# eugenelet/CRFP

Hardware: AMD Instinct MI355X
Metric: sr_frames_per_sec (higher is better)
Workload: dtype f32; 1 GPU; BASELINE configs[1]: single MI355X, 7-frame 180x320 -> 1440x2560 x8 SR, batch=1, fp32, sigma_T=10; mode=clip, frames_per_clip=7, fv_size=96, clips_per_call=1, calls_in_flight_per_gpu=1, clips_in_flight_per_gpu=1, batching=one clip per call, storage=f32, parallelism=clip-sharded x1

## Files before the change

crfp_amd/csrc/engine.hip:

```cpp
#include "crfp_common.h"

#include <cstdlib>
#include <algorithm>
#include <cstring>
#include <mutex>
#include <string>
#include <unordered_map>
#include <vector>

namespace CRFP_NS {

struct ConvDef { const char* stem; int cout, cin; };
constexpr int kNumDsvConvs = 59, kNumCraConvs = 72;
static const ConvDef kConvs[kNumCraConvs] = {
    {"spynet.encoder1.0", 32, 6}, {"spynet.encoder1.2", 32, 32}, {"spynet.encoder2.0", 64, 32},
    {"spynet.encoder2.2", 64, 64}, {"spynet.encoder3.0", 128, 64}, {"spynet.encoder3.2", 128, 128},
    {"spynet.decoder1.0", 256, 128}, {"spynet.decoder1.2", 256, 256}, {"spynet.decoder2.0", 128, 256},
    {"spynet.decoder2.2", 128, 128}, {"spynet.decoder3.0", 64, 128}, {"spynet.decoder3.2", 64, 64},
    {"spynet.flow.0", 32, 64}, {"spynet.flow.2", 2, 32},
    {"dcn_0.dcn_block.0", 32, 66}, {"dcn_0.dcn_block.2", 32, 32}, {"dcn_0.dcn_offset", 144, 32},
    {"dcn_0.dcn_mask", 72, 32}, {"dcn_0.dcn", 32, 32},
    {"dcn_1.conv_fuse", 32, 64}, {"dcn_1.dcn_block.0", 32, 66}, {"dcn_1.dcn_block.2", 32, 32},
    {"dcn_1.dcn_offset", 144, 32}, {"dcn_1.dcn_mask", 72, 32}, {"dcn_1.dcn", 32, 32},
    {"dcn_2.conv_fuse", 32, 64}, {"dcn_2.dcn_block.0", 32, 66}, {"dcn_2.dcn_block.2", 32, 32},
// ... 296 lines not shown
struct Q4 {
    float* p = nullptr;
    int nq = 0, H = 0, W = 0;
    long long bs() const { return (long long)nq * H * W * 4; }
};

constexpr int kFlatFrames = 32, kChunkFrames = 8;

struct Layout {
    Arena A;
    int B, t, h, w;
    bool flat;
    int TC;
    Ten status, state_hr, carry;
    Ten flow_lr, e_lr0, x_lr, lr_q4, lr_keep[2];
    Ten fa0, fa1, fp1, fb0, fb1, fp2, fc0, fc1, fp3, fd0, fd1, fu1, fe0, fe1, fu2, ff0, ff1, fu3, fg0, fg1;
    Ten xin8[2], eh[2], x_hr[2], prop0[2], prop_a, prop_b, flow2[2], flow8[2], prev2, prev2w, prevhrw, carryw, fa, fb, offfeat[3], offmask,
        aligned, y0, y1, up, poff, g0, g1, g2, om3, al3, z0, z1, feat, fg2, sc_prop, sc_cw, sc_al, sc_up, sc_al3;
    Ten c_s1, c_a, c_b, c_lv[2][3], c_y, c_f;
    bool cra;
    int pq;
    Ten gate[2];
    long long gate_b;
    int h1, w1, h2, w2, h3, w3;
    int fnet_cap;
    Ten fpart;

    Layout(int B_, int t_, int h_, int w_, int wiring = W_DSV) : B(B_), t(t_), h(h_), w(w_), cra(wiring == W_CRA), pq(wiring >= W_SIMPLE ? 8 : 6) {
        flat = (long long)B * t <= kFlatFrames;
        TC = flat ? t : kChunkFrames;
        const int nb = t == 1 ? B : (flat ? B * t - 1 : TC);
        fnet_cap = nb;
        const int H2 = 2 * h, W2 = 2 * w, H8 = 8 * h, W8 = 8 * w;
        h1 = h / 2; w1 = w / 2; h2 = h1 / 2; w2 = w1 / 2; h3 = h2 / 2; w3 = w2 / 2;
        status = A.take("status", 1, 0, 1, B > 64 ? (B + 1) / 2 : 32, 1);
        state_hr = A.take("state_hr", B, 1, H8, W8, 0, 1);
        carry = A.take("carry", B, 6, H2, W2, 0, 1);
        flow_lr = A.take("flow_lr", t == 1 ? 2 * B : B * TC, 1, h, w, 0, 0, true);
// ... 25 lines not shown
        {
            const int lh[7] = {h, h1, h2, h3, 2 * h3, 4 * h3, 8 * h3}, lw[7] = {w, w1, w2, w3, 2 * w3, 4 * w3, 8 * w3};
            long long most = 0;
            for (int i = 0; i < 14; ++i) {
                const int kq = (kConvs[i].cin / 4 + 3) / 4 * 4, H = lh[i / 2], W = lw[i / 2];
                const int ks = H > 0 && W > 0 ? conv_auto_ksplit(H, W, (kConvs[i].cout + 31) / 32, kq) : 1;
                if (ks > 1) most = std::max(most, (long long)ks * kConvs[i].cout * H * W);
            }
            const long long per = (long long)h * w * 4;
            fpart = A.take("fnet.part", nb, (int)((most + per - 1) / per), h, w, 0, 0, true);
        }
        for (int p = 0; p < 2; ++p) {
            xin8[p] = A.take(p ? "xin8.1" : "xin8", B, 2, H8, W8);
            eh[p] = A.take(p ? "enc_hr0.1" : "enc_hr0", B, 1, H8, W8);
            x_hr[p] = A.take(p ? "x_hr.1" : "x_hr", B, 1, H8, W8);
            prop0[p] = A.take(p ? "prop0.1" : "prop0", B, pq, H2, W2);
            flow2[p] = A.take(p ? "flow2.1" : "flow2", B, 0, H2, W2, 1);
            flow8[p] = A.take(p ? "flow8.1" : "flow8", B, 0, H8, W8, 1);
            const int gtiles = ((W8 + 63) / 64) * ((H8 + 15) / 16);
            gate_b = ((long long)gtiles * 4 + 7) / 8 * 8;
            gate[p] = A.take(p ? "gate.1" : "gate", B, 0, 1, (int)(gate_b / 8), 1);
        }
        prop_a = A.take("prop_a", B, pq, H2, W2);
        prop_b = A.take("prop_b", B, pq, H2, W2);
        prev2 = A.take("prev2", B, 8, H2, W2, 0, 1);
        prev2w = A.take("prev2w", B, 8, H2, W2);
        prevhrw = A.take("prevhrw", B, 1, H8, W8);
        carryw = A.take("carryw", B, 6, H2, W2);
        fa = A.take("dcn.fa", B, 8, H2, W2);
        fb = A.take("dcn.fb", B, 8, H2, W2);
        for (int l = 0; l < 3; ++l) offfeat[l] = A.take(l == 0 ? "offfeat0" : (l == 1 ? "offfeat1" : "offfeat2"), B, 8, H2, W2);
        offmask = A.take("offmask", B, 54, H2, W2, 0, 0, true);
        aligned = A.take("aligned", B, 8, H2, W2);
        y0 = A.take("res.y0", B, 8, H2, W2);
        y1 = A.take("res.y1", B, 8, H2, W2);
        up = A.take("up", B, 1, H8, W8);
// ... 15 lines not shown
                for (int k = 0; k < 3; ++k) c_lv[p][k] = A.take(lvn[p][k], B, 4, H2, W2);
            c_y = A.take("cra.y", B, 8, H2, W2);
            c_f = A.take("cra.fused", B, 8, H2, W2);
        }
        if (t == 1 && B == 1) {
            fg2 = A.take("fg2", 1, 0, H2 / 2, W2, 1);
            sc_prop = A.take("fg.prop", 1, 6, H2, W2);
            sc_cw = A.take("fg.carry", 1, 2, H2, W2);
            sc_al = A.take("fg.aligned", 1, 8, H2, W2);
            sc_up = A.take("fg.up", 1, 1, H8, W8);
            sc_al3 = A.take("fg.aligned3", 1, 1, H8, W8);
        }
    }
    size_t bytes() const { return A.cur; }
    long long slot(int b, int i) const { return (long long)b * TC + i % TC; }
};

struct StreamCtx {
    unsigned n = 0;
    bool kept = false;
    bool chained = false;
};
struct SideStream {
    hipStream_t s = nullptr;
    std::vector<hipEvent_t> ev;
    std::unordered_map<const void*, StreamCtx> ctx;
    bool ok = true;
    hipEvent_t event(size_t i) {
        while (ev.size() <= i) {
            hipEvent_t e;
// ... 52 lines not shown
    int dev = 0;
    if (hipGetDevice(&dev) != hipSuccess || dev < 0 || dev >= kMaxDevices) return nullptr;
    return &side_table()[dev];
}
static SideStream* side_stream() {
    SideStream* ss = side_slot();
    if (!ss) return nullptr;
    if (!ss->s && ss->ok && hipStreamCreateWithFlags(&ss->s, hipStreamNonBlocking) != hipSuccess) ss->ok = false;
    return ss->ok ? ss : nullptr;
}
static bool side_stream_enabled() {
    static const bool on = !(getenv("CRFP_SIDE_STREAM") && atoi(getenv("CRFP_SIDE_STREAM")) == 0);
    return on;
}

struct Runner {
    const Model& M;
    const float* packed;
    char* ws;
    const Layout& L;
    hipStream_t s;
    int rc = 0;
    int strict = 0;
    bool down_done = false;
    int flow_slot = 0;
    float* flow_lr_slot() const { return F(L.flow_lr) + (long long)flow_slot * L.B * L.h * L.w * 4; }

    int ovf_div = 1, ovf_add = 0, ovf_off = 0, ovf_skip0 = 0;
    unsigned* ovf() const {
        static const bool env_strict = precision_env_strict(0);
// ... 74 lines not shown
        if (rc) return;
        const ConvArgs a = bind(idA, N, H, W, srcsA, {}), b = bind(idB, N, H, W, {{nullptr, 0}}, dstsB, residB, residB_bs);
        rc = launch_conv_pair(a, b, name, s);
    }
#endif
    bool pair_convs() const {
        static const int mode = !kActBf16 ? 0 : (getenv("CRFP_CONV_PAIR") ? atoi(getenv("CRFP_CONV_PAIR")) : 1);
        const long long pair_tiles = (long long)L.B * ((2 * L.w + 61) / 62) * ((2 * L.h + 7) / 8);
        return mode == 2 || (mode == 1 && pair_tiles <= 512);
    }
    void mfma_q(int id, int N, const Q4& in, const Q4& out) {
        mfma(id, N, in.H, in.W, {{in.p, in.bs()}}, {{out.p, out.bs(), 0, out.nq}});
    }
    struct NB { const float* p = nullptr; long long bs = 0; NB() {} NB(const float* p_, long long bs_) : p(p_), bs(bs_) {} };
    void narrow(int id, int H, int W, std::vector<NB> srcs, NB dst, NB resid = NB(), NB flow = NB(), const uint8_t* mask = nullptr,
                long long mask_bs = 0, int src0_pad = 0, int dst_pad = 0, NB base_lr = NB(), int gate_par = -1, int gate_h = 0, NB dst2 = NB()) {
        if (rc) return;
        const Item& it = M.items[id];
        NarrowArgs a = it.nw;
        for (size_t i = 0; i < srcs.size(); ++i) { a.src[i].p = srcs[i].p; a.src[i].bstride = srcs[i].bs; a.src[i].pad = 0; }
        a.src[0].pad = src0_pad;
        a.dst_pad = dst_pad;
        a.N = L.B; a.H = H; a.W = W;
        a.dst = const_cast<float*>(dst.p); a.dst_bstride = dst.bs;
        a.resid = resid.p; a.resid_bstride = resid.bs;
        a.flow = flow.p; a.flow_bstride = flow.bs;
        a.base = nullptr; a.base_lr = base_lr.p; a.base_bstride = base_lr.bs;
        a.mask = mask; a.mask_bstride = mask_bs;
        a.wpk = packed + it.off_w;
        a.bpk = packed + it.off_b;
        a.ovf = ovf(); a.ovf_div = ovf_div; a.ovf_add = ovf_add;
        a.dst2 = const_cast<float*>(dst2.p); a.dst2_bstride = dst2.bs;
        if (gate_par >= 0 && mask_gate_enabled()) { a.gate = gate_ptr(gate_par); a.gate_bstride = L.gate_b; a.gate_h = gate_h; }
        rc = launch_narrow(a, it.name, s);
    }
    void narrow_pair(int idA, int idB, const char* name, int H, int W, std::vector<NB> srcsA, NB dst, NB residB = NB(), NB flowB = NB(), NB dst2B = NB()) {
        if (rc) return;
        NarrowArgs a = M.items[idA].nw, b = M.items[idB].nw;
        for (size_t i = 0; i < srcsA.size(); ++i) { a.src[i].p = srcsA[i].p; a.src[i].bstride = srcsA[i].bs; a.src[i].pad = 0; }
        a.N = b.N = L.B; a.H = b.H = H; a.W = b.W = W;
        a.wpk = packed + M.items[idA].off_w; a.bpk = packed + M.items[idA].off_b;
        b.wpk = packed + M.items[idB].off_w; b.bpk = packed + M.items[idB].off_b;
        b.dst = const_cast<float*>(dst.p); b.dst_bstride = dst.bs;
        b.resid = residB.p; b.resid_bstride = residB.bs;
        b.flow = flowB.p; b.flow_bstride = flowB.bs;
        b.dst_pad = 0;
        b.dst2 = const_cast<float*>(dst2B.p); b.dst2_bstride = dst2B.bs;
        b.ovf = ovf(); b.ovf_div = ovf_div; b.ovf_add = ovf_add;
// ... 33 lines not shown
#endif
#ifdef CRFP_LAB
    static bool state_from_epilogue() {
        static const bool on = getenv("CRFP_STATE_FROM_EPILOGUE") ? atoi(getenv("CRFP_STATE_FROM_EPILOGUE")) != 0 : CRFP_STATE_FROM_EPILOGUE != 0;
        return on;
    }
#else
    static constexpr bool state_from_epilogue() { return CRFP_STATE_FROM_EPILOGUE != 0; }
#endif
#define RUN(expr) do { if (!rc) rc = (expr); } while (0)

    static bool mask_gate_enabled() {
        static const bool on = !(getenv("CRFP_MASK_GATE") && atoi(getenv("CRFP_MASK_GATE")) == 0);
        return on;
    }
    const uint8_t* gate_ptr(int par) const { return reinterpret_cast<const uint8_t*>(ws + L.gate[par]); }

    const float* lr_to_q4(const float* lrs, int n, int s0, int check_div = -1) {
        if (kActBf16) return lrs;
        float* dst = adv(F(L.lr_q4), (long long)s0 * L.h * L.w * 4);
        RUN(launch_nchw_to_q4(lrs, dst, n, 3, L.h, L.w, 0, s, check_div >= 0 ? ovf() : nullptr, check_div));
        return dst;
    }
    long long lr_frame_floats() const { return kActBf16 ? 3LL * L.h * L.w : (long long)L.h * L.w * 4 * (long long)sizeof(act_t) / 4; }
    long long lr_bs(long long nchw_bs) const { return kActBf16 ? nchw_bs : (nchw_bs ? (long long)L.h * L.w * 4 : 0); }

    void fnet(int nb, const float* cur, long long cur_bs, const float* prev, long long prev_bs, float* flow_out, int group = 0) {
        const int h = L.h, w = L.w;
        if (!rc && nb > L.fnet_cap) { set_error("dsv: FNet pass of %d pairs exceeds the workspace's %d", nb, L.fnet_cap); rc = CRFP_E_WORKSPACE; }
        if (rc || nb < 1) return;
        cur_bs = lr_bs(cur_bs); prev_bs = lr_bs(prev_bs);
// ... 38 lines not shown
        pool(conv(5, c0, c1), c1, p3);
        reduce(conv(6, p3, d0), d0);
        resize2(conv(7, d0, d1), d1, u1);
        reduce(conv(8, u1, e0), e0);
        resize2(conv(9, e0, e1), e1, u2);
        reduce(conv(10, u2, f0), f0);
        resize2(conv(11, f0, f1), f1, u3);
        reduce(conv(12, u3, g0), g0);
        mfma(IT_F0 + 13, nb, g0.H, g0.W, {{g0.p, g0.bs()}}, {{g1.p, g1.bs(), 0, g1.nq}}, 0, 0, nullptr, 0, nullptr, 0, nullptr, 0, 1);
        RUN(crfp::launch_upsample_q4(g1.p, g1.bs(), fl.p, fl.bs(), nb, 1, g1.H, g1.W, h, w, (float)g1.H / (float)h,
                                     (float)g1.W / (float)w, 1.0f, s, group));
    }

    void reset_state() {
        if (!rc && hipMemsetAsync(ws + L.status, 0, L.A.find(L.status.off)->bytes, s) != hipSuccess) { set_error("dsv: hipMemsetAsync of the status words failed"); rc = 1; }
        for (size_t off : {L.state_hr.off, L.carry.off, L.prev2.off}) {
            const Buf* b = L.A.find(off);
            if (!rc && hipMemsetAsync(ws + off - b->guard, 0, b->bytes + b->guard, s) != hipSuccess) {
                set_error("dsv: hipMemsetAsync of recurrent state failed");
                rc = 1;
            }
        }
    }

    void encode_lr(int n, const float* lrs, long long bs, long long slot0 = 0) {
        if (rc || n < 1) return;
        const long long xq = 8LL * L.h * L.w * 4;
        Q4 e0 = q(L.e_lr0, 8, L.h, L.w), x = q(L.x_lr, 8, L.h, L.w);
        e0.p = adv(e0.p, slot0 * xq); x.p = adv(x.p, slot0 * xq);
        mfma(IT_ENC_LR0, n, L.h, L.w, {{lrs, lr_bs(bs)}}, {{e0.p, e0.bs(), 0, 8}});
        mfma_q(IT_ENC_LR1, n, e0, x);
    }

    void clip_stage(const float* lq, int i0, int i1, int parts) {
        const long long lqf = lr_frame_floats(), lr_f = 3LL * L.h * L.w, fq = (long long)L.h * L.w * 4;
        const int t = L.t, B = L.B;
        struct Restore { Runner& r; int d, a, o; ~Restore() { r.ovf_div = d; r.ovf_add = a; r.ovf_off = o; r.ovf_skip0 = 0; } } restore{*this, ovf_div, ovf_add, ovf_off};
// ... 46 lines not shown
        const float* x_lr = nullptr; long long x_b = 0;
    };
    FrameIO frame_io(int i, const float* lrs, const float* fvs, const uint8_t* mks, float* out, int y_only) const {
        const long long lr_f = 3LL * L.h * L.w, hr_px = 64LL * L.h * L.w, xq = 8LL * L.h * L.w * 4, fq = (long long)L.h * L.w * 4;
        const int co = y_only ? 1 : 3, t = L.t;
        FrameIO f;
        f.lr = lrs + i * lr_f; f.lr_b = t * lr_f;
        f.fv = fvs + i * 3 * hr_px; f.fv_b = t * 3 * hr_px;
        f.mk = mks + i * hr_px; f.mk_b = t * hr_px;
        f.out = out + (long long)i * co * hr_px; f.out_b = (long long)t * co * hr_px;
        f.flow_lr = i > 0 ? F(L.flow_lr) + L.slot(0, i) * fq : nullptr; f.flow_b = L.TC * fq;
        f.x_lr = adv(F(L.x_lr), L.slot(0, i) * xq); f.x_b = L.TC * xq;
        return f;
    }

    void frame_pre(int par, bool first, const FrameIO& io, hipEvent_t before_ups = nullptr, int parts = 3) {
        const int h = L.h, w = L.w, H2 = 2 * h, W2 = 2 * w, H8 = 8 * h, W8 = 8 * w, B = L.B;
        const long long P8q = (long long)H8 * W8 * 4;
        if (parts & 1) {
            const Ten& xin = L.xin8[par];
            const bool gated = mask_gate_enabled();
            if (gated) RUN(launch_mask_gate(io.mk, io.mk_b, const_cast<uint8_t*>(gate_ptr(par)), L.gate_b, B, H8, W8, s));
            const int gp = (gated && !M.cra && !(pair_mask() & 1)) ? par : -1;
            RUN(launch_hr_prep(io.lr, io.fv, io.mk, F(xin), h, w, s, B, io.lr_b, io.fv_b, io.mk_b, xin.bs, gp >= 0 ? gate_ptr(par) : nullptr, L.gate_b));
            const Ten& s1 = M.cra ? L.c_s1 : L.x_hr[par];
            if (pair_mask() & 1)
                narrow_pair(IT_EH0, IT_EH1, "conv_narrow_pair:enc_hr", H8, W8, {{F(xin), xin.bs}, {adv(F(xin), P8q), xin.bs}}, {F(s1), s1.bs});
            else {
                narrow(IT_EH0, H8, W8, {{F(xin), xin.bs}, {adv(F(xin), P8q), xin.bs}}, {F(L.eh[par]), L.eh[par].bs}, NB(), NB(), nullptr, 0, 0, 0, NB(), gp, 2);
                narrow(IT_EH1, H8, W8, {{F(L.eh[par]), L.eh[par].bs}}, {F(s1), s1.bs}, NB(), NB(), nullptr, 0, 0, 0, NB(), gp, 1);
            }
            if (M.cra) {
                narrow(IT_C_LV3, H8, W8, {{F(s1), s1.bs}}, {F(L.x_hr[par]), L.x_hr[par].bs}, NB(), NB(), nullptr, 0, 0, 0, NB(), par, 1);
                const Q4 a = q(L.c_a, 4, H2, W2), b = q(L.c_b, 4, H2, W2);
                auto lv = [&](int k) { return q(L.c_lv[par][k], 4, H2, W2); };
                mfma(IT_C_S2A, B, H2, W2, {{F(s1), s1.bs, 0}}, {{a.p, a.bs(), 0, 4}});
                mfma_q(IT_C_S2B, B, a, b);
                mfma_q(IT_C_LV2, B, b, lv(2));
                mfma_q(IT_C_S3A, B, b, a);
                mfma_q(IT_C_S3B, B, a, b);
                mfma_q(IT_C_LV1, B, b, lv(1));
                mfma_q(IT_C_S4A, B, b, a);
                mfma_q(IT_C_S4B, B, a, b);
                mfma_q(IT_C_LV0, B, b, lv(0));
            }
            if (before_ups && !rc && hipStreamWaitEvent(s, before_ups, 0) != hipSuccess) { set_error("dsv: hipStreamWaitEvent failed"); rc = 1; }
            mfma(IT_UPS, B, h, w, {{io.x_lr, io.x_b}}, {{F(L.prop0[par]), L.prop0[par].bs, 0, L.pq}}, H2, W2);
        }
        if (!first && (parts & 2)) {
            RUN(crfp::launch_upflow(io.flow_lr, io.flow_b, F(L.flow2[par]), L.flow2[par].bs, B, h, w, 2, s));
            RUN(crfp::launch_upflow(io.flow_lr, io.flow_b, F(L.flow8[par]), L.flow8[par].bs, B, h, w, 8, s));
        }
    }

    void downsample_state() {
        mfma(IT_DOWN, L.B, 2 * L.h, 2 * L.w, {{F(L.state_hr), L.state_hr.bs, 1}}, {{F(L.prev2), L.prev2.bs, 0, 8, 1}});
    }

    void frame(int par, bool first, const FrameIO& io, const uint8_t* fg = nullptr) {
        const int h = L.h, w = L.w, H2 = 2 * h, W2 = 2 * w, H8 = 8 * h, W8 = 8 * w, B = L.B;
        const long long P2q = (long long)H2 * W2 * 4;
        const long long P2qp = (long long)(H2 + 1) * (W2 + 1) * 4;
        const long long bs8 = 8 * P2q;
        const long long bs6 = L.pq * P2q;
        const bool abl = M.abl(), dense = M.dense();
        float* prop = F(L.prop0[par]);
        float* prop_next = F(L.prop_a);
        float* prop_other = F(L.prop_b);
        float* carry = F(L.carry);
        auto nb = [&](const Ten& tn) { return NB(F(tn), tn.bs); };
        std::vector<NB> r3_srcs;
        const bool r3_chain = (chain_mask() & 2) && !(kActBf16 && dense && !first);
        if (!first) {
            float* flow2 = F(L.flow2[par]);
            float* flow8 = F(L.flow8[par]);
            const long long f2b = L.flow2[par].bs, f8b = L.flow8[par].bs;
            if (!down_done) downsample_state();
            if (abl) {
                RUN(launch_flow_warp_q4(F(L.state_hr), L.state_hr.bs, flow8, f8b, F(L.prevhrw), L.prevhrw.bs, B, 1, H8, W8, 0, 1, s));
                mfma(IT_DOWN, B, H2, W2, {{F(L.prevhrw), L.prevhrw.bs, 0}}, {{F(L.prev2w), L.prev2w.bs, 0, 8}});
            } else {
            WarpDualStrides wb;
            wb.xa = L.prev2.bs; wb.xb = L.carry.bs; wb.flow = f2b; wb.outa = L.prev2w.bs; wb.outb = L.carryw.bs;
            RUN(launch_flow_warp_p4_dual_8_6(F(L.prev2), carry, flow2, F(L.prev2w), F(L.carryw), H2, W2, s, B, wb));
            RUN(launch_flow_warp_q4(F(L.state_hr), L.state_hr.bs, flow8, f8b, F(L.prevhrw), L.prevhrw.bs, B, 1, H8, W8, 0, 1, s));
            }
            const float* offprev = nullptr;
            if (fg) RUN(crfp::launch_fg_prep(fg, F(L.fg2), H8, W8, s));
            for (int l = 0; l < 3; ++l) {
                const float* cw = adv(F(L.carryw), 2 * l * P2q);
                float* f = F(L.offfeat[l]);
                const bool s3 = M.use_s3;
                const std::vector<SrcBind> db0 = abl ? std::vector<SrcBind>{{prop, bs6}, {F(L.prev2w), bs8}, {flow2, f2b}, {nullptr, 0}}
                                                     : std::vector<SrcBind>{{prop, bs6}, {cw, bs6}, {F(L.prev2w), bs8}, {flow2, f2b}, {nullptr, 0}};
#ifdef CRFP_ACT_BF16
                if (pair_convs())
                    mfma_pair(it_lvl(l, L_DB0), it_lvl(l, L_DB1), "conv_mfma_pair:dcn.block0_block2", B, H2, W2, db0, {{l == 0 ? f : F(L.fb), bs8, 0, 8}});
                else
#endif
                {
                mfma(it_lvl(l, L_DB0), B, H2, W2, db0, {{F(L.fa), bs8, 0, 8}});
                if (l == 0) {
                    if (s3) mfma(it_lvl(l, L_DB1), B, H2, W2, {{F(L.fa), bs8}}, {}, 0, 0, nullptr, 0, nullptr, 0, f, bs8);
                    else mfma(it_lvl(l, L_DB1), B, H2, W2, {{F(L.fa), bs8}}, {{f, bs8, 0, 8}});
                } else
                    mfma(it_lvl(l, L_DB1), B, H2, W2, {{F(L.fa), bs8}}, {{F(L.fb), bs8, 0, 8}});
                }
                if (l > 0) {
                    if (s3) mfma(it_lvl(l, L_FUSE), B, H2, W2, {{F(L.fb), bs8}, {offprev, bs8}}, {}, 0, 0, nullptr, 0, nullptr, 0, f, bs8);
// ... 10 lines not shown
                    fa.x = F(L.prev2); fa.xb = L.prev2.bs;
                    fa.wdcn = packed + dw.off_w + 36 * 2 * 32 * 4; fa.bdcn = packed + dw.off_b;
                    fa.out = F(L.aligned); fa.ob = bs8; fa.N = B; fa.H = H2; fa.W = W2; fa.ovf = ovf(); fa.ovf_div = ovf_div;
                    RUN(launch_dcn_fused(fa, s));
                } else {
                    mfma(it_lvl(l, L_OM), B, H2, W2, {{f, bs8}}, {{F(L.offmask), L.offmask.bs, 0, 54}}, 0, 0, nullptr, 0, flow2, f2b);
                    RUN(launch_dcn_g8(F(L.prev2), L.prev2.bs, F(L.offmask), L.offmask.bs, packed + dw.off_w + (f16 ? 36 * 2 * 32 * 4 : 0), packed + dw.off_b,
                                      F(L.aligned), bs8, B, H2, W2, s, f16, ovf(), ovf_div));
                }
                if (fg && l > 0) {
                    RUN(launch_scale_q4(prop, 0, F(L.sc_prop), 6, H2, W2, F(L.fg2), nullptr, s));
                    RUN(launch_scale_q4(cw, 0, F(L.sc_cw), 2, H2, W2, F(L.fg2), nullptr, s));
                    RUN(launch_scale_q4(F(L.aligned), 0, F(L.sc_al), 8, H2, W2, F(L.fg2), nullptr, s));
                    mfma(it_lvl(l, L_RB0), 1, H2, W2, {{F(L.sc_prop), 0}, {F(L.sc_cw), 0}, {F(L.sc_al), 0}}, {{F(L.y0), 0, 0, 8}});
                } else if (abl) {
                    std::vector<SrcBind> rb = {{prop, bs6}, {F(L.aligned), bs8}};
                    if (dense) rb.push_back({F(L.prev2w), bs8});
                    mfma(it_lvl(l, L_RB0), B, H2, W2, rb, {{F(L.y0), bs8, 0, 8}});
                } else
                    mfma(it_lvl(l, L_RB0), B, H2, W2, {{prop, bs6}, {cw, bs6}, {F(L.aligned), bs8}}, {{F(L.y0), bs8, 0, 8}});
                res_block(l, prop_next, adv(carry, 2 * l * P2qp), H2, W2, par, io.mk, io.mk_b);
                prop = prop_next;
                std::swap(prop_next, prop_other);
                offprev = f;
            }
            mfma_dual(IT_UPP, {{prop, bs6}}, {{F(L.up), L.up.bs, 0, 1}}, IT_POFF, {{offprev, bs8}}, {{F(L.poff), L.poff.bs, 0, 1}}, B, H2, W2, H8, W8,
                      "conv_mfma:upsample_post_ps4+dcn3.preoffset_ps4");
            const NB fl8(flow8, f8b);
            if (chain_mask() & 1)
                narrow_chain(IT_D3B0, IT_D3B1, IT_D3FUSE, "conv_narrow_chain:dcn3.block0_block2_fuse", H8, W8, {nb(L.up), nb(L.prevhrw), fl8}, nb(L.poff),
                             nb(L.g2), false);
            else {
            if (pair_mask() & 8)
                narrow_pair(IT_D3B0, IT_D3B1, "conv_narrow_pair:dcn3.block", H8, W8, {nb(L.up), nb(L.prevhrw), fl8}, nb(L.g1));
            else {
                narrow(IT_D3B0, H8, W8, {nb(L.up), nb(L.prevhrw), fl8}, nb(L.g0));
                narrow(IT_D3B1, H8, W8, {nb(L.g0)}, nb(L.g1));
            }
            if (pair_mask() & 2)
                narrow_pair(IT_D3FUSE, IT_D3OM, "conv_narrow_pair:dcn3.fuse_offmask", H8, W8, {nb(L.g1), nb(L.poff)}, nb(L.om3), NB(), fl8);
            else
// ... 6 lines not shown
                                      packed + d3.off_b, F(L.al3), L.al3.bs, B, H8, W8, s, f8b));
            } else {
                if (!(pair_mask() & 2)) narrow(IT_D3OM, H8, W8, {nb(L.g2)}, nb(L.om3), NB(), fl8);
                RUN(launch_dcn3(F(L.state_hr), L.state_hr.bs, F(L.om3), L.om3.bs, packed + d3.off_w, packed + d3.off_b, F(L.al3), L.al3.bs, B, H8, W8, s));
            }
            if (fg) {
                RUN(launch_scale_q4(F(L.up), 0, F(L.sc_up), 1, H8, W8, nullptr, fg, s));
                RUN(launch_scale_q4(F(L.al3), 0, F(L.sc_al3), 1, H8, W8, nullptr, fg, s));
                r3_srcs = {nb(L.sc_up), nb(L.sc_al3)};
            } else
                r3_srcs = {nb(L.up), nb(L.al3)};
            if (dense) r3_srcs.push_back(nb(L.prevhrw));
            if (!r3_chain) narrow(IT_R3_0, H8, W8, r3_srcs, nb(L.z0));
        } else {
            for (int l = 0; l < 3; ++l) {
                mfma(it_lvl(l, L_RB0F), B, H2, W2, {{prop, bs6}, {nullptr, 0}}, {{F(L.y0), bs8, 0, 8}});
                res_block(l, prop_next, adv(carry, 2 * l * P2qp), H2, W2, par, io.mk, io.mk_b);
                prop = prop_next;
                std::swap(prop_next, prop_other);
            }
            mfma(IT_UPP, B, H2, W2, {{prop, bs6}}, {{F(L.up), L.up.bs, 0, 1}}, H8, W8);
            r3_srcs = {nb(L.up)};
            if (!r3_chain) narrow(IT_R3_0F, H8, W8, r3_srcs, nb(L.z0));
        }
        const NB st2 = mask_gate_enabled() && state_from_epilogue() ? nb(L.state_hr) : NB();
        if (r3_chain)
            narrow_chain(first ? IT_R3_0F : IT_R3_0, IT_R3_1, IT_R3_2, "conv_narrow_chain:res3.main0_conv1_conv2_add", H8, W8, r3_srcs, NB(), nb(L.feat), true, st2);
        else if (pair_mask() & 4)
            narrow_pair(IT_R3_1, IT_R3_2, "conv_narrow_pair:res3.conv1_conv2_add", H8, W8, {nb(L.z0)}, nb(L.feat), nb(L.z0), NB(), st2);
        else {
            narrow(IT_R3_1, H8, W8, {nb(L.z0)}, nb(L.z1));
            narrow(IT_R3_2, H8, W8, {nb(L.z1)}, nb(L.feat), nb(L.z0), NB(), nullptr, 0, 0, 0, NB(), -1, 0, st2);
        }
        if (mask_gate_enabled() && !st2.p) RUN(launch_lrelu_q4_to_p4(F(L.feat), L.feat.bs, F(L.state_hr), L.state_hr.bs, B, H8, W8, ovf(), ovf_div, s));
        narrow(IT_TTTF, H8, W8, {nb(L.feat), nb(L.x_hr[par])}, nb(L.state_hr), NB(), NB(), io.mk, io.mk_b, 0, 1, NB(), par, 0);
        narrow(IT_LAST, H8, W8, {nb(L.state_hr)}, NB(io.out, io.out_b), NB(), NB(), nullptr, 0, 1, 0, NB(io.lr, io.lr_b));
    }
};

}

using namespace CRFP_NS;

#ifdef CRFP_ACT_BF16
__global__ void round_bf16_copy_kernel(const float* __restrict__ src, float* __restrict__ dst, int n) {
    const int i = blockIdx.x * blockDim.x + threadIdx.x;
    if (i < n) dst[i] = (float)(__bf16)src[i];
}
namespace crfp_bf16 { void shutdown_side_streams() { destroy_all_side_streams(); } }
#else
// ... 155 lines not shown

static int forward_batch_impl(int wiring, const void* packed, int flags, const float* lrs, const float* fvs, const uint8_t* mks,
                              float* out, int n, int t, int h, int w, void* workspace, size_t workspace_bytes, void* stream) {
    const int y_only = flags & CRFP_DSV_Y_ONLY;
    if (kActBf16 && (flags & CRFP_DSV_STRICT_F32)) { set_error("dsv (bf16 storage): CRFP_DSV_STRICT_F32 belongs to the fp32 entry points"); return CRFP_E_UNSUPPORTED; }
    if (!dims_ok(n, t, h, w)) { set_error("dsv: need n,t>=1, h,w>=8 (got %d,%d,%d,%d)", n, t, h, w); return CRFP_E_BADARG; }
    Layout L(n, t, h, w, wiring);
    int rc = check_common(packed, n, t, h, w, workspace, workspace_bytes, L);
    if (rc) return rc;
    if (!lrs || !fvs || !mks || !out) { set_error("dsv_forward_clip: null tensor"); return CRFP_E_BADARG; }
    Runner R{model_for(y_only, flags & CRFP_DSV_STRICT_F32, wiring), (const float*)packed, (char*)workspace, L, (hipStream_t)stream};
    R.strict = (flags & CRFP_DSV_STRICT_F32) ? 1 : 0;
    const int TC = L.TC;
    SideStream* ssp = side_stream_enabled() && !prof_enabled() && !(flags & CRFP_DSV_SINGLE_STREAM) ? side_stream() : nullptr;
    hipStream_t main_s = (hipStream_t)stream;
    if (!ssp) {
        R.reset_state();
        const float* lq = R.lr_to_q4(lrs, n * t, 0, t);
        for (int i = 0; i < t && !R.rc; ++i) {
            if (i % TC == 0) {
                const int i1 = i + TC < t ? i + TC : t;
                R.clip_stage(lq, i, i1, 2);
                R.clip_stage(lq, i, i1, 1);
            }
            const Runner::FrameIO io = R.frame_io(i, lrs, fvs, mks, out, y_only);
            R.frame_pre(i & 1, i == 0, io);
            R.frame(i & 1, i == 0, io);
        }
        return R.rc;
    }
    SideStream& ss = *ssp;
    bool forked = false;
    auto join = [&]() {
        hipEvent_t ej = ss.event(0);
        if (forked && ej && hipEventRecord(ej, ss.s) == hipSuccess) (void)hipStreamWaitEvent(main_s, ej, 0);
    };
    auto fail = [&](const char* what) { join(); set_error("dsv_forward_clip: %s failed", what); return 1; };
    hipEvent_t ev_start = ss.event(0), ev_xlr = ss.event(1);
    if (!ss.ok) return fail("hipEventCreate");
    R.reset_state();
    const float* lq = R.lr_to_q4(lrs, n * t, 0, t);
    if (R.rc) return R.rc;
    if (hipEventRecord(ev_start, main_s) != hipSuccess || hipStreamWaitEvent(ss.s, ev_start, 0) != hipSuccess) return fail("fork");
    forked = true;
    R.clip_stage(lq, 0, TC < t ? TC : t, 1);
    if (hipEventRecord(ev_xlr, main_s) != hipSuccess) return fail("record");
    for (int i = 0; i < t && !R.rc; ++i) {
        hipEvent_t pre_done = ss.event(2 + 2 * i), main_done = ss.event(3 + 2 * i);
        if (!ss.ok) return fail("hipEventCreate");
        R.s = ss.s;
        if (i == 1) R.clip_stage(lq, 0, TC < t ? TC : t, 2);
        if (i > 0 && i % TC == 0) R.clip_stage(lq, i, i + TC < t ? i + TC : t, 3);
        if (i >= 2 && hipStreamWaitEvent(ss.s, ss.event(3 + 2 * (i - 2)), 0) != hipSuccess) return fail("wait");
        const Runner::FrameIO io = R.frame_io(i, lrs, fvs, mks, out, y_only);
        R.frame_pre(i & 1, i == 0, io, i == 0 ? ev_xlr : nullptr);
        if (hipEventRecord(pre_done, ss.s) != hipSuccess) return fail("record");
        R.s = main_s;
        if (hipStreamWaitEvent(main_s, pre_done, 0) != hipSuccess) return fail("wait");
        R.frame(i & 1, i == 0, io);
        if (hipEventRecord(main_done, main_s) != hipSuccess) return fail("record");
    }
    if (R.rc) join();
    return R.rc;
}

extern "C" {

int CRFP_API(crfp_dsv_forward_batch)(const void* packed, int flags, const float* lrs, const float* fvs, const uint8_t* mks,
                           float* out, int n, int t, int h, int w, void* workspace, size_t workspace_bytes, void* stream) {
    return forward_batch_impl(W_DSV, packed, flags, lrs, fvs, mks, out, n, t, h, w, workspace, workspace_bytes, stream);
}

int CRFP_API(crfp_cra_forward_batch)(const void* packed, int flags, const float* lrs, const float* fvs, const uint8_t* mks,
                           float* out, int n, int t, int h, int w, void* workspace, size_t workspace_bytes, void* stream) {
// ... 231 lines not shown
```

Before: 711.4 frames/s.

## Batch per-clip mask gate, LR upsample and flow upsample across frames

Gives prop0, flow2 and the mask gate one slot per frame instead of two ping-pong slots. Their producers (mask gate, UPS conv, 2x flow upsample) now run as a single launch over all frames of a chunk rather than once per frame, which cuts launch count and raises per-kernel parallelism at 180x320. Reset also swaps three full-buffer memsets of the recurrent state for one kernel that zeroes only the pad borders and guards. The cost is more workspace and changed side-stream ordering, and state interiors are no longer zeroed, so correctness depends on those regions being fully written before they are read.

```diff
diff --git a/crfp_amd/csrc/engine.hip b/crfp_amd/csrc/engine.hip
--- a/crfp_amd/csrc/engine.hip
+++ b/crfp_amd/csrc/engine.hip
@@ -334,14 +334,14 @@
     int TC;
     Ten status, state_hr, carry;
     Ten flow_lr, e_lr0, x_lr, lr_q4, lr_keep[2];
+    Ten prop0, flow2, gate;
+    long long gate_b;
     Ten fa0, fa1, fp1, fb0, fb1, fp2, fc0, fc1, fp3, fd0, fd1, fu1, fe0, fe1, fu2, ff0, ff1, fu3, fg0, fg1;
-    Ten xin8[2], eh[2], x_hr[2], prop0[2], prop_a, prop_b, flow2[2], flow8[2], prev2, prev2w, prevhrw, carryw, fa, fb, offfeat[3], offmask,
+    Ten xin8[2], eh[2], x_hr[2], prop_a, prop_b, flow8[2], prev2, prev2w, prevhrw, carryw, fa, fb, offfeat[3], offmask,
         aligned, y0, y1, up, poff, g0, g1, g2, om3, al3, z0, z1, feat, fg2, sc_prop, sc_cw, sc_al, sc_up, sc_al3;
     Ten c_s1, c_a, c_b, c_lv[2][3], c_y, c_f;
     bool cra;
     int pq;
-    Ten gate[2];
-    long long gate_b;
     int h1, w1, h2, w2, h3, w3;
     int fnet_cap;
     Ten fpart;
@@ -397,12 +397,15 @@
             xin8[p] = A.take(p ? "xin8.1" : "xin8", B, 2, H8, W8);
             eh[p] = A.take(p ? "enc_hr0.1" : "enc_hr0", B, 1, H8, W8);
             x_hr[p] = A.take(p ? "x_hr.1" : "x_hr", B, 1, H8, W8);
-            prop0[p] = A.take(p ? "prop0.1" : "prop0", B, pq, H2, W2);
-            flow2[p] = A.take(p ? "flow2.1" : "flow2", B, 0, H2, W2, 1);
             flow8[p] = A.take(p ? "flow8.1" : "flow8", B, 0, H8, W8, 1);
+        }
+        {
+            const int slots = t == 1 ? 2 * B : B * TC;
+            prop0 = A.take("prop0", slots, pq, H2, W2);
+            flow2 = A.take("flow2", slots, 0, H2, W2, 1);
             const int gtiles = ((W8 + 63) / 64) * ((H8 + 15) / 16);
             gate_b = ((long long)gtiles * 4 + 7) / 8 * 8;
-            gate[p] = A.take(p ? "gate.1" : "gate", B, 0, 1, (int)(gate_b / 8), 1);
+            gate = A.take("gate", slots, 0, 1, (int)(gate_b / 8), 1);
         }
         prop_a = A.take("prop_a", B, pq, H2, W2);
         prop_b = A.take("prop_b", B, pq, H2, W2);
@@ -448,6 +451,8 @@
     }
     size_t bytes() const { return A.cur; }
     long long slot(int b, int i) const { return (long long)b * TC + i % TC; }
+    long long pre_slot(int k) const { return t == 1 ? (long long)k * B : k % TC; }
+    long long pre_stride() const { return t == 1 ? 1 : TC; }
 };
 
 struct StreamCtx {
@@ -530,6 +535,21 @@
     return on;
 }
 
+struct PadClear { act_t* p; int planes, H, W, guard; };
+struct PadClearArgs { PadClear b[3]; };
+__global__ void clear_p4_pads_kernel(const PadClearArgs a) {
+    const PadClear c = a.b[blockIdx.y];
+    const long long per = (long long)c.H + c.W + 1;
+    long long i = (long long)blockIdx.x * blockDim.x + threadIdx.x;
+    const cf32x4 zero = cf32x4{0.0f, 0.0f, 0.0f, 0.0f};
+    if (i < c.guard) { stq(c.p - 4 * (c.guard - i), zero); return; }
+    i -= c.guard;
+    if (i >= per * c.planes) return;
+    const long long plane = i / per, k = i - plane * per, row = c.W + 1;
+    const long long q = plane * (c.H + 1) * row + (k < c.H ? k * row + c.W : (long long)c.H * row + (k - c.H));
+    stq(c.p + 4 * q, zero);
+}
+
 struct Runner {
     const Model& M;
     const float* packed;
@@ -634,7 +654,7 @@
     }
     struct NB { const float* p = nullptr; long long bs = 0; NB() {} NB(const float* p_, long long bs_) : p(p_), bs(bs_) {} };
     void narrow(int id, int H, int W, std::vector<NB> srcs, NB dst, NB resid = NB(), NB flow = NB(), const uint8_t* mask = nullptr,
-                long long mask_bs = 0, int src0_pad = 0, int dst_pad = 0, NB base_lr = NB(), int gate_par = -1, int gate_h = 0, NB dst2 = NB()) {
+                long long mask_bs = 0, int src0_pad = 0, int dst_pad = 0, NB base_lr = NB(), int gate_key = -1, int gate_h = 0, NB dst2 = NB()) {
         if (rc) return;
         const Item& it = M.items[id];
         NarrowArgs a = it.nw;
@@ -651,7 +671,7 @@
         a.bpk = packed + it.off_b;
         a.ovf = ovf(); a.ovf_div = ovf_div; a.ovf_add = ovf_add;
         a.dst2 = const_cast<float*>(dst2.p); a.dst2_bstride = dst2.bs;
-        if (gate_par >= 0 && mask_gate_enabled()) { a.gate = gate_ptr(gate_par); a.gate_bstride = L.gate_b; a.gate_h = gate_h; }
+        if (gate_key >= 0 && mask_gate_enabled()) { a.gate = gate_ptr(gate_key); a.gate_bstride = gate_bs(); a.gate_h = gate_h; }
         rc = launch_narrow(a, it.name, s);
     }
     void narrow_pair(int idA, int idB, const char* name, int H, int W, std::vector<NB> srcsA, NB dst, NB residB = NB(), NB flowB = NB(), NB dst2B = NB()) {
@@ -715,7 +735,20 @@
         static const bool on = !(getenv("CRFP_MASK_GATE") && atoi(getenv("CRFP_MASK_GATE")) == 0);
         return on;
     }
-    const uint8_t* gate_ptr(int par) const { return reinterpret_cast<const uint8_t*>(ws + L.gate[par]); }
+    const uint8_t* gate_ptr(int k) const { return reinterpret_cast<const uint8_t*>(ws + L.gate) + L.pre_slot(k) * L.gate_b; }
+    long long gate_bs() const { return L.pre_stride() * L.gate_b; }
+    float* prop0_ptr(int k) const { return adv(F(L.prop0), L.pre_slot(k) * L.prop0.bs); }
+    long long prop0_bs() const { return L.pre_stride() * L.prop0.bs; }
+    float* flow2_ptr(int k) const { return F(L.flow2) + L.pre_slot(k) * L.flow2.bs; }
+    long long flow2_bs() const { return L.pre_stride() * L.flow2.bs; }
+#ifdef CRFP_LAB
+    static bool clip_pre_batch_enabled() {
+        static const bool on = !(getenv("CRFP_CLIP_PRE_BATCH") && atoi(getenv("CRFP_CLIP_PRE_BATCH")) == 0);
+        return on;
+    }
+#else
+    static constexpr bool clip_pre_batch_enabled() { return true; }
+#endif
 
     const float* lr_to_q4(const float* lrs, int n, int s0, int check_div = -1) {
         if (kActBf16) return lrs;
@@ -784,13 +817,18 @@
 
     void reset_state() {
         if (!rc && hipMemsetAsync(ws + L.status, 0, L.A.find(L.status.off)->bytes, s) != hipSuccess) { set_error("dsv: hipMemsetAsync of the status words failed"); rc = 1; }
+        if (rc) return;
+        PadClearArgs a;
+        long long most = 0;
+        int k = 0;
         for (size_t off : {L.state_hr.off, L.carry.off, L.prev2.off}) {
             const Buf* b = L.A.find(off);
-            if (!rc && hipMemsetAsync(ws + off - b->guard, 0, b->bytes + b->guard, s) != hipSuccess) {
-                set_error("dsv: hipMemsetAsync of recurrent state failed");
-                rc = 1;
-            }
-        }
+            a.b[k] = PadClear{as_act(F(off)), b->N * b->nq, b->H, b->W, (int)(b->guard / kQuadBytes)};
+            most = std::max(most, a.b[k].guard + (long long)a.b[k].planes * (b->H + b->W + 1));
+            ++k;
+        }
+        clear_p4_pads_kernel<<<dim3((unsigned)((most + 255) / 256), 3), 256, 0, s>>>(a);
+        if (hipGetLastError() != hipSuccess) { set_error("dsv: launch of clear_p4_pads_kernel failed"); rc = 1; }
     }
 
     void encode_lr(int n, const float* lrs, long long bs, long long slot0 = 0) {
@@ -867,15 +905,40 @@
         return f;
     }
 
-    void frame_pre(int par, bool first, const FrameIO& io, hipEvent_t before_ups = nullptr, int parts = 3) {
+    void pre_batch(const uint8_t* mks, int i0, int i1, int parts) {
+        const int h = L.h, w = L.w, H8 = 8 * h, W8 = 8 * w, t = L.t;
+        const long long hr_px = 64LL * h * w, xq = 8LL * h * w * 4, fq = (long long)h * w * 4;
+        if (rc || i1 <= i0) return;
+        struct Restore { Runner& r; int d, a, o; ~Restore() { r.ovf_div = d; r.ovf_add = a; r.ovf_off = o; } } restore{*this, ovf_div, ovf_add, ovf_off};
+        ovf_div = 0;
+        ovf_add = 0;
+        for (int b = 0; b < L.B && !rc; ++b) {
+            ovf_off = b;
+            const long long s0 = L.slot(b, i0);
+            if (parts & 1) {
+                if (mask_gate_enabled())
+                    RUN(launch_mask_gate(mks + ((long long)b * t + i0) * hr_px, hr_px, reinterpret_cast<uint8_t*>(ws + L.gate) + s0 * L.gate_b, L.gate_b, i1 - i0,
+                                         H8, W8, s));
+                mfma(IT_UPS, i1 - i0, h, w, {{adv(F(L.x_lr), s0 * xq), xq}}, {{adv(F(L.prop0), s0 * L.prop0.bs), L.prop0.bs, 0, L.pq}}, 2 * h, 2 * w);
+            }
+            const int j0 = i0 > 0 ? i0 : 1;
+            if ((parts & 2) && i1 > j0) {
+                const long long sj = L.slot(b, j0);
+                RUN(crfp::launch_upflow(F(L.flow_lr) + sj * fq, fq, F(L.flow2) + sj * L.flow2.bs, L.flow2.bs, i1 - j0, h, w, 2, s));
+            }
+        }
+    }
+
+    void frame_pre(int par, bool first, const FrameIO& io, hipEvent_t before_ups = nullptr, int parts = 3, int key = -1, bool batched = false) {
         const int h = L.h, w = L.w, H2 = 2 * h, W2 = 2 * w, H8 = 8 * h, W8 = 8 * w, B = L.B;
         const long long P8q = (long long)H8 * W8 * 4;
+        if (key < 0) key = par;
         if (parts & 1) {
             const Ten& xin = L.xin8[par];
             const bool gated = mask_gate_enabled();
-            if (gated) RUN(launch_mask_gate(io.mk, io.mk_b, const_cast<uint8_t*>(gate_ptr(par)), L.gate_b, B, H8, W8, s));
-            const int gp = (gated && !M.cra && !(pair_mask() & 1)) ? par : -1;
-            RUN(launch_hr_prep(io.lr, io.fv, io.mk, F(xin), h, w, s, B, io.lr_b, io.fv_b, io.mk_b, xin.bs, gp >= 0 ? gate_ptr(par) : nullptr, L.gate_b));
+            if (gated && !batched) RUN(launch_mask_gate(io.mk, io.mk_b, const_cast<uint8_t*>(gate_ptr(key)), gate_bs(), B, H8, W8, s));
+            const int gp = (gated && !M.cra && !(pair_mask() & 1)) ? key : -1;
+            RUN(launch_hr_prep(io.lr, io.fv, io.mk, F(xin), h, w, s, B, io.lr_b, io.fv_b, io.mk_b, xin.bs, gp >= 0 ? gate_ptr(key) : nullptr, gate_bs()));
             const Ten& s1 = M.cra ? L.c_s1 : L.x_hr[par];
             if (pair_mask() & 1)
                 narrow_pair(IT_EH0, IT_EH1, "conv_narrow_pair:enc_hr", H8, W8, {{F(xin), xin.bs}, {adv(F(xin), P8q), xin.bs}}, {F(s1), s1.bs});
@@ -884,7 +947,7 @@
                 narrow(IT_EH1, H8, W8, {{F(L.eh[par]), L.eh[par].bs}}, {F(s1), s1.bs}, NB(), NB(), nullptr, 0, 0, 0, NB(), gp, 1);
             }
             if (M.cra) {
-                narrow(IT_C_LV3, H8, W8, {{F(s1), s1.bs}}, {F(L.x_hr[par]), L.x_hr[par].bs}, NB(), NB(), nullptr, 0, 0, 0, NB(), par, 1);
+                narrow(IT_C_LV3, H8, W8, {{F(s1), s1.bs}}, {F(L.x_hr[par]), L.x_hr[par].bs}, NB(), NB(), nullptr, 0, 0, 0, NB(), key, 1);
                 const Q4 a = q(L.c_a, 4, H2, W2), b = q(L.c_b, 4, H2, W2);
                 auto lv = [&](int k) { return q(L.c_lv[par][k], 4, H2, W2); };
                 mfma(IT_C_S2A, B, H2, W2, {{F(s1), s1.bs, 0}}, {{a.p, a.bs(), 0, 4}});
@@ -898,10 +961,10 @@
                 mfma_q(IT_C_LV0, B, b, lv(0));
             }
             if (before_ups && !rc && hipStreamWaitEvent(s, before_ups, 0) != hipSuccess) { set_error("dsv: hipStreamWaitEvent failed"); rc = 1; }
-            mfma(IT_UPS, B, h, w, {{io.x_lr, io.x_b}}, {{F(L.prop0[par]), L.prop0[par].bs, 0, L.pq}}, H2, W2);
+            if (!batched) mfma(IT_UPS, B, h, w, {{io.x_lr, io.x_b}}, {{prop0_ptr(key), prop0_bs(), 0, L.pq}}, H2, W2);
         }
         if (!first && (parts & 2)) {
-            RUN(crfp::launch_upflow(io.flow_lr, io.flow_b, F(L.flow2[par]), L.flow2[par].bs, B, h, w, 2, s));
+            if (!batched) RUN(crfp::launch_upflow(io.flow_lr, io.flow_b, flow2_ptr(key), flow2_bs(), B, h, w, 2, s));
             RUN(crfp::launch_upflow(io.flow_lr, io.flow_b, F(L.flow8[par]), L.flow8[par].bs, B, h, w, 8, s));
         }
     }
@@ -910,14 +973,16 @@
         mfma(IT_DOWN, L.B, 2 * L.h, 2 * L.w, {{F(L.state_hr), L.state_hr.bs, 1}}, {{F(L.prev2), L.prev2.bs, 0, 8, 1}});
     }
 
-    void frame(int par, bool first, const FrameIO& io, const uint8_t* fg = nullptr) {
+    void frame(int par, bool first, const FrameIO& io, const uint8_t* fg = nullptr, int key = -1) {
         const int h = L.h, w = L.w, H2 = 2 * h, W2 = 2 * w, H8 = 8 * h, W8 = 8 * w, B = L.B;
         const long long P2q = (long long)H2 * W2 * 4;
         const long long P2qp = (long long)(H2 + 1) * (W2 + 1) * 4;
         const long long bs8 = 8 * P2q;
         const long long bs6 = L.pq * P2q;
         const bool abl = M.abl(), dense = M.dense();
-        float* prop = F(L.prop0[par]);
+        if (key < 0) key = par;
+        float* prop = prop0_ptr(key);
+        long long pbs = prop0_bs();
         float* prop_next = F(L.prop_a);
         float* prop_other = F(L.prop_b);
         float* carry = F(L.carry);
@@ -925,9 +990,9 @@
         std::vector<NB> r3_srcs;
         const bool r3_chain = (chain_mask() & 2) && !(kActBf16 && dense && !first);
         if (!first) {
-            float* flow2 = F(L.flow2[par]);
+            float* flow2 = flow2_ptr(key);
             float* flow8 = F(L.flow8[par]);
-            const long long f2b = L.flow2[par].bs, f8b = L.flow8[par].bs;
+            const long long f2b = flow2_bs(), f8b = L.flow8[par].bs;
             if (!down_done) downsample_state();
             if (abl) {
                 RUN(launch_flow_warp_q4(F(L.state_hr), L.state_hr.bs, flow8, f8b, F(L.prevhrw), L.prevhrw.bs, B, 1, H8, W8, 0, 1, s));
@@ -944,8 +1009,8 @@
                 const float* cw = adv(F(L.carryw), 2 * l * P2q);
                 float* f = F(L.offfeat[l]);
                 const bool s3 = M.use_s3;
-                const std::vector<SrcBind> db0 = abl ? std::vector<SrcBind>{{prop, bs6}, {F(L.prev2w), bs8}, {flow2, f2b}, {nullptr, 0}}
-                                                     : std::vector<SrcBind>{{prop, bs6}, {cw, bs6}, {F(L.prev2w), bs8}, {flow2, f2b}, {nullptr, 0}};
+                const std::vector<SrcBind> db0 = abl ? std::vector<SrcBind>{{prop, pbs}, {F(L.prev2w), bs8}, {flow2, f2b}, {nullptr, 0}}
+                                                     : std::vector<SrcBind>{{prop, pbs}, {cw, bs6}, {F(L.prev2w), bs8}, {flow2, f2b}, {nullptr, 0}};
 #ifdef CRFP_ACT_BF16
                 if (pair_convs())
                     mfma_pair(it_lvl(l, L_DB0), it_lvl(l, L_DB1), "conv_mfma_pair:dcn.block0_block2", B, H2, W2, db0, {{l == 0 ? f : F(L.fb), bs8, 0, 8}});
@@ -986,17 +1051,18 @@
                     RUN(launch_scale_q4(F(L.aligned), 0, F(L.sc_al), 8, H2, W2, F(L.fg2), nullptr, s));
                     mfma(it_lvl(l, L_RB0), 1, H2, W2, {{F(L.sc_prop), 0}, {F(L.sc_cw), 0}, {F(L.sc_al), 0}}, {{F(L.y0), 0, 0, 8}});
                 } else if (abl) {
-                    std::vector<SrcBind> rb = {{prop, bs6}, {F(L.aligned), bs8}};
+                    std::vector<SrcBind> rb = {{prop, pbs}, {F(L.aligned), bs8}};
                     if (dense) rb.push_back({F(L.prev2w), bs8});
                     mfma(it_lvl(l, L_RB0), B, H2, W2, rb, {{F(L.y0), bs8, 0, 8}});
                 } else
-                    mfma(it_lvl(l, L_RB0), B, H2, W2, {{prop, bs6}, {cw, bs6}, {F(L.aligned), bs8}}, {{F(L.y0), bs8, 0, 8}});
+                    mfma(it_lvl(l, L_RB0), B, H2, W2, {{prop, pbs}, {cw, bs6}, {F(L.aligned), bs8}}, {{F(L.y0), bs8, 0, 8}});
                 res_block(l, prop_next, adv(carry, 2 * l * P2qp), H2, W2, par, io.mk, io.mk_b);
                 prop = prop_next;
+                pbs = bs6;
                 std::swap(prop_next, prop_other);
                 offprev = f;
             }
-            mfma_dual(IT_UPP, {{prop, bs6}}, {{F(L.up), L.up.bs, 0, 1}}, IT_POFF, {{offprev, bs8}}, {{F(L.poff), L.poff.bs, 0, 1}}, B, H2, W2, H8, W8,
+            mfma_dual(IT_UPP, {{prop, pbs}}, {{F(L.up), L.up.bs, 0, 1}}, IT_POFF, {{offprev, bs8}}, {{F(L.poff), L.poff.bs, 0, 1}}, B, H2, W2, H8, W8,
                       "conv_mfma:upsample_post_ps4+dcn3.preoffset_ps4");
             const NB fl8(flow8, f8b);
             if (chain_mask() & 1)
@@ -1033,12 +1099,13 @@
             if (!r3_chain) narrow(IT_R3_0, H8, W8, r3_srcs, nb(L.z0));
         } else {
             for (int l = 0; l < 3; ++l) {
-                mfma(it_lvl(l, L_RB0F), B, H2, W2, {{prop, bs6}, {nullptr, 0}}, {{F(L.y0), bs8, 0, 8}});
+                mfma(it_lvl(l, L_RB0F), B, H2, W2, {{prop, pbs}, {nullptr, 0}}, {{F(L.y0), bs8, 0, 8}});
                 res_block(l, prop_next, adv(carry, 2 * l * P2qp), H2, W2, par, io.mk, io.mk_b);
                 prop = prop_next;
+                pbs = bs6;
                 std::swap(prop_next, prop_other);
             }
-            mfma(IT_UPP, B, H2, W2, {{prop, bs6}}, {{F(L.up), L.up.bs, 0, 1}}, H8, W8);
+            mfma(IT_UPP, B, H2, W2, {{prop, pbs}}, {{F(L.up), L.up.bs, 0, 1}}, H8, W8);
             r3_srcs = {nb(L.up)};
             if (!r3_chain) narrow(IT_R3_0F, H8, W8, r3_srcs, nb(L.z0));
         }
@@ -1052,7 +1119,7 @@
             narrow(IT_R3_2, H8, W8, {nb(L.z1)}, nb(L.feat), nb(L.z0), NB(), nullptr, 0, 0, 0, NB(), -1, 0, st2);
         }
         if (mask_gate_enabled() && !st2.p) RUN(launch_lrelu_q4_to_p4(F(L.feat), L.feat.bs, F(L.state_hr), L.state_hr.bs, B, H8, W8, ovf(), ovf_div, s));
-        narrow(IT_TTTF, H8, W8, {nb(L.feat), nb(L.x_hr[par])}, nb(L.state_hr), NB(), NB(), io.mk, io.mk_b, 0, 1, NB(), par, 0);
+        narrow(IT_TTTF, H8, W8, {nb(L.feat), nb(L.x_hr[par])}, nb(L.state_hr), NB(), NB(), io.mk, io.mk_b, 0, 1, NB(), key, 0);
         narrow(IT_LAST, H8, W8, {nb(L.state_hr)}, NB(io.out, io.out_b), NB(), NB(), nullptr, 0, 1, 0, NB(io.lr, io.lr_b));
     }
 };
@@ -1238,6 +1305,7 @@
     const int TC = L.TC;
     SideStream* ssp = side_stream_enabled() && !prof_enabled() && !(flags & CRFP_DSV_SINGLE_STREAM) ? side_stream() : nullptr;
     hipStream_t main_s = (hipStream_t)stream;
+    const bool batch = Runner::clip_pre_batch_enabled();
     if (!ssp) {
         R.reset_state();
         const float* lq = R.lr_to_q4(lrs, n * t, 0, t);
@@ -1246,10 +1314,11 @@
                 const int i1 = i + TC < t ? i + TC : t;
                 R.clip_stage(lq, i, i1, 2);
                 R.clip_stage(lq, i, i1, 1);
+                if (batch) R.pre_batch(mks, i, i1, 3);
             }
             const Runner::FrameIO io = R.frame_io(i, lrs, fvs, mks, out, y_only);
-            R.frame_pre(i & 1, i == 0, io);
-            R.frame(i & 1, i == 0, io);
+            R.frame_pre(i & 1, i == 0, io, nullptr, 3, i, batch);
+            R.frame(i & 1, i == 0, io, nullptr, i);
         }
         return R.rc;
     }
@@ -1273,15 +1342,19 @@
         hipEvent_t pre_done = ss.event(2 + 2 * i), main_done = ss.event(3 + 2 * i);
         if (!ss.ok) return fail("hipEventCreate");
         R.s = ss.s;
-        if (i == 1) R.clip_stage(lq, 0, TC < t ? TC : t, 2);
-        if (i > 0 && i % TC == 0) R.clip_stage(lq, i, i + TC < t ? i + TC : t, 3);
+        const int i1 = i - i % TC + TC < t ? i - i % TC + TC : t;
+        if (i == 1 && batch) R.pre_batch(mks, 1, i1, 1);
+        if (i == 1) R.clip_stage(lq, 0, i1, 2);
+        if (i == 1 && batch) R.pre_batch(mks, 1, i1, 2);
+        if (i > 0 && i % TC == 0) R.clip_stage(lq, i, i1, 3);
         if (i >= 2 && hipStreamWaitEvent(ss.s, ss.event(3 + 2 * (i - 2)), 0) != hipSuccess) return fail("wait");
+        if (i > 1 && i % TC == 1 && batch) R.pre_batch(mks, i, i1, 3);
         const Runner::FrameIO io = R.frame_io(i, lrs, fvs, mks, out, y_only);
-        R.frame_pre(i & 1, i == 0, io, i == 0 ? ev_xlr : nullptr);
+        R.frame_pre(i & 1, i == 0, io, i == 0 ? ev_xlr : nullptr, 3, i, batch && i % TC != 0);
         if (hipEventRecord(pre_done, ss.s) != hipSuccess) return fail("record");
         R.s = main_s;
         if (hipStreamWaitEvent(main_s, pre_done, 0) != hipSuccess) return fail("wait");
-        R.frame(i & 1, i == 0, io);
+        R.frame(i & 1, i == 0, io, nullptr, i);
         if (hipEventRecord(main_done, main_s) != hipSuccess) return fail("record");
     }
     if (R.rc) join();
```

Measured after the change: 713.6 frames/s (median of 6 runs). Within noise of the previous version (+0.3%).
